# keras-team/keras-rs

Measured on AMD Instinct MI355X. Metric: embedding lookups/sec + DCN fwd+bwd step time, 26-table DLRM batch 65 536, higher is better.
Workload: dtype bf16; 1 GPU; C3 DLRM-small: 26 tables x 1000000 rows x 128 (bf16), global batch 65536, multi-hot ml_perf lengths (sum L = 214), uniform ids, DotInteraction(F=27) + 3 x FeatureCross(d=3456, projection=512), fused Adagrad on tables; global_batch=65536, parallelism=single GPU

## Files before the change

include/krs.h:

```cpp
#ifndef KRS_H_
#define KRS_H_

#include <stddef.h>
#include <stdint.h>

#ifdef __cplusplus
extern "C" {
#endif

#define KRS_VERSION 100

typedef enum krs_status {
  KRS_OK = 0,
  KRS_ERR_INVALID = -1,
  KRS_ERR_UNSUPPORTED = -2,
  KRS_ERR_LAUNCH = -3,
  KRS_ERR_WORKSPACE = -4
} krs_status;

typedef enum krs_dtype { KRS_F32 = 0, KRS_BF16 = 1 } krs_dtype;
typedef enum krs_itype { KRS_I32 = 0, KRS_I64 = 1 } krs_itype;

typedef enum krs_combiner { KRS_SUM = 0, KRS_MEAN = 1, KRS_SQRTN = 2 } krs_combiner;

// ... 147 lines not shown
enum { KRS_CROSS_BWD_NONE = 0, KRS_CROSS_BWD_TWO_CALL = 1, KRS_CROSS_BWD_PP64 = 2, KRS_CROSS_BWD_PP256 = 3 };
int krs_gemm_cross_bwd_last_route(int* epilogue);

enum {
  KRS_GEMM_KERNEL_NONE = 0, KRS_GEMM_KERNEL_GENERIC = 1, KRS_GEMM_KERNEL_MFMA = 2, KRS_GEMM_KERNEL_GLDS = 3,
  KRS_GEMM_KERNEL_TN_GLDS = 4, KRS_GEMM_KERNEL_PP256 = 5, KRS_GEMM_KERNEL_PP256_KSTRIDED = 6, KRS_GEMM_KERNEL_PP64 = 7,
  KRS_GEMM_KERNEL_THIN = 8, KRS_GEMM_KERNEL_ROWDOT = 9, KRS_GEMM_KERNEL_SMALLK = 10
};
enum { KRS_GEMM_REDUCE_NONE = 0, KRS_GEMM_REDUCE_SCALAR = 1, KRS_GEMM_REDUCE_VEC4 = 2, KRS_GEMM_REDUCE_VEC8 = 3 };
typedef struct krs_gemm_route {
  int32_t kernel;
  int32_t splits;
  int32_t reduce;
  int32_t epilogue;
  int32_t ep_vec;
  int32_t thin_width;
  int32_t thin_is_a;
} krs_gemm_route;
int krs_gemm_last_route(krs_gemm_route* route);

enum { KRS_GEMM_OPT_PIPELINE = 0 };
int krs_gemm_set_option(int key, int value);

enum { KRS_EMBED_OPT_PLAN = 2, KRS_EMBED_OPT_HOTROWS = 3, KRS_EMBED_OPT_RANK = 4 };
int krs_embed_set_option(int key, int value);

size_t krs_colsum_workspace_bytes(int64_t m, int64_t n);
int krs_cross_epilogue_fwd(const void* u, const void* x0, const void* x, void* y,
                           int64_t m, int64_t n, int64_t ld, float diag_scale,
                           int dtype, void* stream);
int krs_cross_epilogue_bwd(const void* g, const void* u, const void* x0, const void* x,
                           void* du, void* dx0, int dx0_accumulate, void* dxd,
                           float* dbias,
                           int64_t m, int64_t n, int64_t ld, float diag_scale, int act,
                           int dtype, void* workspace, size_t workspace_bytes, void* stream);

int krs_cast_transpose(const void* src, int64_t rows, int64_t cols, int64_t ld_src, int src_dtype,
                       void* dst, int64_t ld_dst, void* dst_t, int64_t ld_dst_t, int dst_dtype,
                       void* stream);
int krs_cast_transpose_many(int count, const void* const* srcs, const int64_t* rows, const int64_t* cols,
                            int src_dtype, void* const* dsts, void* const* dst_ts, int dst_dtype, void* stream);

int krs_dense_act_bwd(const void* g, int64_t ld_g, const void* y, int64_t ld_y, void* dz, int64_t ld_dz,
                      float* dbias, int64_t m, int64_t n, int act, int dtype, void* workspace,
                      size_t workspace_bytes, void* stream);

int krs_dense_adagrad(float* const* params, const float* const* grads, float* const* accs,
// ... 133 lines not shown
```

keras_rs_amd/csrc/embed_bag_fwd.hip:

```cpp
#include <cstdlib>

#include "krs_common.h"

namespace krs {
namespace {

typedef uint32_t u32x4 __attribute__((ext_vector_type(4)));
typedef float f32x4 __attribute__((ext_vector_type(4)));
constexpr int NT = 2;

struct EmbedFwdParams {
  const krs_table* tables;
  const krs_feature* feats;
  int n_feats;
  const void* ids;
  int id64;
  const void* offsets;
  int off64;
  const float* weights;
  int batch;
  int dim;
  void* out;
  int64_t out_ld;
  float* bag_scale;
// ... 522 lines not shown
      }
      KRS_CHECK_LAUNCH("embed_bag_fwd_vec (hot rows in LDS)");
      return KRS_OK;
    }
  }
  if (p.weights) { if (stream) KRS_K1_LAUNCH(true, true); else KRS_K1_LAUNCH(true, false); }
  else { if (stream) KRS_K1_LAUNCH(false, true); else KRS_K1_LAUNCH(false, false); }
#undef KRS_K1_LAUNCH
  KRS_CHECK_LAUNCH("embed_bag_fwd_vec");
  return KRS_OK;
}

template <typename TT, typename OT>
int dispatch_lpr(const EmbedFwdParams& p, int row_pieces, bool one_hot, bool stream_mode, hipStream_t stream) {
  if (row_pieces <= 8) return launch_vec<TT, OT, 8>(p, one_hot, stream_mode, stream);
  if (row_pieces <= 16) return launch_vec<TT, OT, 16>(p, one_hot, stream_mode, stream);
  if (row_pieces <= 32) return launch_vec<TT, OT, 32>(p, one_hot, stream_mode, stream);
  return launch_vec<TT, OT, 64>(p, one_hot, stream_mode, stream);
}

}
}

namespace krs { extern int g_plan_variant, g_rank_mode; }

extern "C" int krs_embed_set_option(int key, int value) {
  if (key == KRS_EMBED_OPT_PLAN) {
    KRS_REQUIRE(value == 0 || value == 1, "krs_embed_set_option: plan variant must be 0 or 1");
    krs::g_plan_variant = value;
    return KRS_OK;
  }
  if (key == KRS_EMBED_OPT_RANK) {
    KRS_REQUIRE(value >= 0 && value <= 2, "krs_embed_set_option: rank mode must be 0, 1 or 2");
    krs::g_rank_mode = value;
    return KRS_OK;
  }
  if (key == KRS_EMBED_OPT_HOTROWS) {
    KRS_REQUIRE(value == 0 || value == 64 || value == 128, "krs_embed_set_option: hot rows must be 0, 64 or 128");
    krs::g_hot_rows = value;
    return KRS_OK;
  }
  return krs::fail(KRS_ERR_INVALID, "krs_embed_set_option: unknown key %d", key);
}

extern "C" int krs_embed_bag_fwd(const krs_table* tables, const krs_feature* feats, int n_feats,
                                 const void* ids, int id_type, const void* offsets, int off_type,
                                 const float* weights, int64_t nnz, int batch, int dim,
                                 int table_dtype, void* out, int out_dtype, int64_t out_ld,
                                 float* bag_scale, int* err_flag, void* stream) {
  using namespace krs;
  KRS_REQUIRE(tables && feats && out, "embed_bag_fwd: null tables/feats/out");
  KRS_REQUIRE(ids || nnz == 0, "embed_bag_fwd: null ids");
  KRS_REQUIRE(n_feats >= 0 && batch >= 0 && dim > 0 && nnz >= 0, "embed_bag_fwd: negative size");
  KRS_REQUIRE((table_dtype == KRS_F32 || table_dtype == KRS_BF16) &&
                  (out_dtype == KRS_F32 || out_dtype == KRS_BF16),
              "embed_bag_fwd: bad dtype");
  KRS_REQUIRE((id_type == KRS_I32 || id_type == KRS_I64) && (off_type == KRS_I32 || off_type == KRS_I64),
// ... 37 lines not shown
```

keras_rs_amd/csrc/embed_bag_plan.hip:

```cpp
#include <algorithm>

#include "krs_bag_plan.h"

namespace krs {
int g_plan_variant = 0;
int g_rank_mode = 0;
namespace {

namespace rs {
constexpr int kHistThreads = 256, kHistItems = kTile / kHistThreads;
constexpr int kThreads = 512, kWaves = kThreads / 64, kItems = kTile / kThreads;
constexpr int kGenFeats = 256;

struct Gen {
  const krs_table* tables;
  const krs_feature* feats;
  int n_feats;
  const void* ids;
  int id64;
  int batch;
  int* err_flag;
};

struct alignas(16) GenLds {
  uint32_t base[kGenFeats + 1];
  uint32_t hot[kGenFeats];
  uint32_t row_base[kGenFeats];
  uint32_t vocab[kGenFeats];
};
__device__ __forceinline__ void load_gen(const Gen& gen, int64_t nnz, GenLds& g, int n_threads) {
  for (int i = threadIdx.x; i <= gen.n_feats; i += n_threads) {
    if (i < gen.n_feats) {
      const krs_feature ft = gen.feats[i];
      const krs_table tb = gen.tables[ft.table];
      g.base[i] = (uint32_t)ft.ids_base;
      g.hot[i] = (uint32_t)ft.hot;
      g.row_base[i] = (uint32_t)tb.row_base;
      g.vocab[i] = (uint32_t)tb.vocab;
    } else {
      g.base[i] = (uint32_t)nnz;
    }
  }
}
__device__ __forceinline__ int gen_feature(const GenLds& g, int n_feats, uint32_t q) {
  int lo = 0, hi = n_feats;
  while (hi - lo > 1) {
    const int mid = (lo + hi) >> 1;
    if (g.base[mid] <= q) lo = mid; else hi = mid;
  }
  return lo;
}
__device__ __forceinline__ uint64_t gen_value(const Gen& gen, const GenLds& g, int f, uint32_t q) {
  const uint32_t bag = (uint32_t)f * (uint32_t)gen.batch + (q - g.base[f]) / g.hot[f];
  return ((uint64_t)bag << 32) | (uint64_t)q;
}
__device__ __forceinline__ bool generate(const Gen& gen, const GenLds& g, uint32_t q, uint32_t& key, uint64_t& val) {
  const int f = gen_feature(g, gen.n_feats, q);
  const int64_t id = ld_index(gen.ids, gen.id64, q);
  const bool valid = id >= 0 && id < (int64_t)g.vocab[f];
  key = valid ? g.row_base[f] + (uint32_t)id : kInvalidKey;
  val = gen_value(gen, g, f, q);
  return valid;
}

__device__ __forceinline__ int digit_of(uint32_t key, int shift, int bins) { return (int)((key >> shift) & (bins - 1)); }

__device__ __forceinline__ uint32_t tile_of_block(uint32_t b, uint32_t tiles) { return (b & 7) * ((tiles + 7) / 8) + (b >> 3); }
inline unsigned tile_grid(unsigned tiles) { return (tiles + 7) / 8 * 8; }

__device__ __forceinline__ void hist_zero(int (&h)[kMaxBins], int bins) {
  for (int i = threadIdx.x; i < bins; i += kHistThreads) h[i] = 0;
}
__device__ __forceinline__ void hist_add(int (&h)[kMaxBins], uint32_t key, int shift, int bins) {
  atomicAdd(&h[digit_of(key, shift, bins)], 1);
}
__device__ __forceinline__ void hist_finish(const int (&h)[kMaxBins], int bins, int32_t* col, int64_t stride, bool bad,
                                            int* err_flag) {
  if (bad && err_flag) atomicOr(err_flag, KRS_FLAG_ID_OUT_OF_RANGE);
  __syncthreads();
  for (int i = threadIdx.x; i < bins; i += kHistThreads) col[(int64_t)i * stride] = h[i];
}

template <typename V>
struct alignas(16) TileLds {
  uint16_t cnt[kWaves][kMaxBins];
  uint16_t tile_excl[kMaxBins];
  int gbase[kMaxBins];
  uint32_t skey[kTile];
  V sval[kTile];
  int wtot[kWaves];
};
template <typename V>
__device__ __forceinline__ void zero_counts(TileLds<V>& s) {
  for (int i = threadIdx.x; i < kWaves * kMaxBins; i += kThreads) (&s.cnt[0][0])[i] = 0;
}
__device__ __forceinline__ unsigned long long digit_peers(int d, bool live, int bits) {
  unsigned long long peers = __ballot(live);
  for (int b = 0; b < bits; ++b) {
    const unsigned long long m = __ballot((d >> b) & 1);
    peers &= ((d >> b) & 1) ? m : ~m;
  }
  return peers;
}
__device__ __forceinline__ int ballot_rank(uint32_t key, bool live, int shift, int bits, volatile uint16_t* mine,
                                           int lane) {
  const int d = digit_of(key, shift, 1 << bits);
  const unsigned long long peers = digit_peers(d, live, bits);
  int r = 0, c = 0;
  if (live) {
    r = __popcll(peers & ((1ULL << lane) - 1ULL));
    const int leader = __ffsll((long long)peers) - 1;
    if (lane == leader) {
      c = mine[d];
      mine[d] = (uint16_t)(c + __popcll(peers));
    }
    c = __shfl(c, leader, 64);
  }
  __builtin_amdgcn_wave_barrier();
  return c + r;
}
typedef uint32_t __attribute__((may_alias)) cnt_word;
__device__ __forceinline__ void count_rank(const uint32_t (&key)[kItems], int64_t first, int64_t end, int shift, int bits,
                                           bool fallback, uint16_t* mine, int lane, int (&rank)[kItems]) {
  cnt_word* word = reinterpret_cast<cnt_word*>(mine);
  uint32_t before[kItems], after[kItems];
#pragma unroll
  for (int it = 0; it < kItems; ++it) {
    const int d = digit_of(key[it], shift, 1 << bits);
// ... 18 lines not shown
    if (fallback && __popcll(pend) / 2 > bits) {
      r = c + __popcll(digit_peers(d, live, bits) & below);
    } else {
      while (pend) {
        const int leader = __ffsll((long long)pend) - 1;
        const int dl = __builtin_amdgcn_readlane(d, leader);
        const unsigned long long peers = __ballot(live && d == dl);
        if (d == dl) r = c + __popcll(peers & below);
        pend &= ~peers;
      }
    }
    rank[it] = live ? r : 0;
  }
}
__device__ __forceinline__ void rank_keys(const uint32_t (&key)[kItems], int64_t first, int64_t end, int shift, int bits,
                                          int mode, uint16_t* mine, int lane, int (&rank)[kItems]) {
  if (mode == 1) {
#pragma unroll
    for (int it = 0; it < kItems; ++it) rank[it] = ballot_rank(key[it], first + it * 64 < end, shift, bits, mine, lane);
  } else {
    count_rank(key, first, end, shift, bits, mode == 0, mine, lane, rank);
  }
}
template <typename V>
__device__ __forceinline__ void digit_bases(TileLds<V>& s, int bins, const int32_t* col, int64_t stride) {
  const int lane = threadIdx.x & 63, wave = threadIdx.x >> 6;
  __syncthreads();
  int tot[2], run = 0;
#pragma unroll
  for (int k = 0; k < 2; ++k) {
    const int i = threadIdx.x * 2 + k;
    tot[k] = 0;
    if (i < bins)
      for (int w = 0; w < kWaves; ++w) tot[k] += s.cnt[w][i];
    run += tot[k];
  }
  int x = run;
#pragma unroll
  for (int o = 1; o < 64; o <<= 1) {
    const int y = __shfl_up(x, o, 64);
    if (lane >= o) x += y;
  }
  if (lane == 63) s.wtot[wave] = x;
  __syncthreads();
  int excl = x - run;
  for (int w = 0; w < wave; ++w) excl += s.wtot[w];
#pragma unroll
  for (int k = 0; k < 2; ++k) {
    const int i = threadIdx.x * 2 + k;
    if (i < bins) {
      s.tile_excl[i] = (uint16_t)excl;
      s.gbase[i] = col[(int64_t)i * stride];
      int o = excl;
      for (int w = 0; w < kWaves; ++w) {
        const int t = s.cnt[w][i];
        s.cnt[w][i] = (uint16_t)o;
        o += t;
      }
      excl += tot[k];
    }
  }
  __syncthreads();
}
template <typename V>
__device__ __forceinline__ void stage_tile(TileLds<V>& s, const uint32_t (&key)[kItems], const V (&val)[kItems],
                                           const int (&rank)[kItems], int64_t first, int64_t end, int shift, int bins) {
  const int wave = threadIdx.x >> 6;
#pragma unroll
  for (int it = 0; it < kItems; ++it) {
    if (first + it * 64 < end) {
      const int lp = s.cnt[wave][digit_of(key[it], shift, bins)] + rank[it];
      s.skey[lp] = key[it];
      s.sval[lp] = val[it];
    }
  }
  __syncthreads();
}
template <typename V>
__device__ __forceinline__ int out_slot(const TileLds<V>& s, int i, int d) {
  return s.gbase[d] + (i - (int)s.tile_excl[d]);
}

struct Pass {
  const uint32_t* keys_in;
  const uint64_t* vals_in;
  uint32_t* keys_out;
  uint64_t* vals_out;
  int32_t* counts;
  int64_t nnz;
  int n_tiles;
  int shift, bits;
  int rank;
  Gen gen;
};

template <bool GEN>
__global__ __launch_bounds__(kHistThreads) void hist_kernel(const Pass p) {
  __shared__ int h[kMaxBins];
  __shared__ GenLds g;
  const uint32_t tile = tile_of_block(blockIdx.x, p.n_tiles);
  if (tile >= (uint32_t)p.n_tiles) return;
  const int bins = 1 << p.bits;
  hist_zero(h, bins);
  if constexpr (GEN) load_gen(p.gen, p.nnz, g, kHistThreads);
  __syncthreads();
  const int64_t base = (int64_t)tile * kTile;
  bool bad = false;
  for (int it = 0; it < kHistItems; ++it) {
    const int64_t q = base + it * kHistThreads + threadIdx.x;
    if (q < p.nnz) {
      uint32_t key;
      if constexpr (GEN) {
        uint64_t v;
        bad |= !generate(p.gen, g, (uint32_t)q, key, v);
      } else {
        key = p.keys_in[q];
      }
      hist_add(h, key, p.shift, bins);
    }
  }
  hist_finish(h, bins, p.counts + tile, p.n_tiles, bad, p.gen.err_flag);
}

template <bool GEN>
__global__ __launch_bounds__(kThreads) void scatter_kernel(const Pass p) {
  __shared__ TileLds<uint64_t> s;
  __shared__ GenLds g;
  const uint32_t tile = tile_of_block(blockIdx.x, p.n_tiles);
  if (tile >= (uint32_t)p.n_tiles) return;
  const int bins = 1 << p.bits;
  zero_counts(s);
  if constexpr (GEN) load_gen(p.gen, p.nnz, g, kThreads);
  __syncthreads();
  const int lane = threadIdx.x & 63, wave = threadIdx.x >> 6;
  const int64_t tile0 = (int64_t)tile * kTile;
  const int64_t first = tile0 + (int64_t)wave * (kTile / kWaves) + lane;
  uint32_t key[kItems];
  uint64_t val[kItems];
  int rank[kItems];
#pragma unroll
  for (int it = 0; it < kItems; ++it) {
    const int64_t q = first + it * 64;
    const bool live = q < p.nnz;
    key[it] = kInvalidKey;
    val[it] = 0;
    if (live) {
      if constexpr (GEN) {
        generate(p.gen, g, (uint32_t)q, key[it], val[it]);
      } else {
        key[it] = p.keys_in[q];
        val[it] = p.vals_in[q];
      }
    }
  }
  rank_keys(key, first, p.nnz, p.shift, p.bits, p.rank, s.cnt[wave], lane, rank);
  digit_bases(s, bins, p.counts + tile, p.n_tiles);
  stage_tile(s, key, val, rank, first, p.nnz, p.shift, bins);
  const int n_here = (int)min<int64_t>(kTile, p.nnz - tile0);
#pragma unroll
  for (int it = 0; it < kItems; ++it) {
    const int i = it * kThreads + threadIdx.x;
    if (i < n_here) {
      const uint32_t k = s.skey[i];
      const int pos = out_slot(s, i, digit_of(k, p.shift, bins));
      p.keys_out[pos] = k;
      p.vals_out[pos] = s.sval[i];
    }
  }
}

struct Seg {
  int n;
  uint32_t lookup_start[kMaxProb + 1];
  uint32_t tile_start[kMaxProb + 1];
  uint32_t row_base[kMaxProb];
};
struct SegPass {
  const uint32_t* keys_in;
  const uint32_t* pos_in;
  uint32_t* keys_out;
  uint32_t* pos_out;
  uint64_t* vals_out;
  int32_t* counts;
  int64_t nnz;
  int shift, bits, key_bits;
  int rank;
  Gen gen;
  Seg seg;
};
struct SegTile {
  int pr;
  int64_t t0, end;
  int32_t* col;
  uint32_t stride;
};
__device__ __forceinline__ SegTile seg_tile(const SegPass& p, uint32_t tile) {
  const Seg& sg = p.seg;
  int lo = 0, hi = sg.n;
  while (hi - lo > 1) {
    const int mid = (lo + hi) >> 1;
    if (sg.tile_start[mid] <= tile) lo = mid; else hi = mid;
  }
  SegTile t;
  t.pr = lo;
  const uint32_t tl = tile - sg.tile_start[lo];
  t.stride = sg.tile_start[lo + 1] - sg.tile_start[lo];
  t.t0 = (int64_t)sg.lookup_start[lo] + (int64_t)tl * kTile;
  t.end = min<int64_t>(t.t0 + kTile, sg.lookup_start[lo + 1]);
  t.col = p.counts + ((int64_t)1 << p.bits) * sg.tile_start[lo] + tl;
  return t;
}
template <int ITEMS, int STRIDE>
__device__ __forceinline__ bool seg_first_keys(const SegPass& p, const GenLds& g, const SegTile& t, int64_t first,
                                               uint32_t (&key)[ITEMS], uint32_t (&pos)[ITEMS]) {
  int64_t idv[ITEMS];
#pragma unroll
  for (int it = 0; it < ITEMS; ++it) idv[it] = ld_index(p.gen.ids, p.gen.id64, min<int64_t>(first + it * STRIDE, t.end - 1));
  const int f_lo = gen_feature(g, p.gen.n_feats, (uint32_t)t.t0), f_hi = gen_feature(g, p.gen.n_feats, (uint32_t)(t.end - 1));
  bool bad = false;
#pragma unroll
  for (int it = 0; it < ITEMS; ++it) {
    const int64_t q = min<int64_t>(first + it * STRIDE, t.end - 1);
    const int f = f_lo == f_hi ? f_lo : gen_feature(g, p.gen.n_feats, (uint32_t)q);
    const bool valid = idv[it] >= 0 && idv[it] < (int64_t)g.vocab[f];
    key[it] = valid ? (uint32_t)idv[it] : (1u << p.key_bits) - 1u;
    pos[it] = (uint32_t)q;
    bad = bad || (!valid && first + it * STRIDE < t.end);
  }
  return bad;
}

template <bool FIRST>
__global__ __launch_bounds__(kHistThreads) void hist_seg_kernel(const SegPass p) {
  __shared__ int h[kMaxBins];
  __shared__ GenLds g;
  const uint32_t tile = tile_of_block(blockIdx.x, p.seg.tile_start[p.seg.n]);
  if (tile >= p.seg.tile_start[p.seg.n]) return;
  const int bins = 1 << p.bits;
  hist_zero(h, bins);
  if constexpr (FIRST) load_gen(p.gen, p.nnz, g, kHistThreads);
  __syncthreads();
  const SegTile t = seg_tile(p, tile);
  const int64_t first = t.t0 + threadIdx.x;
  bool bad = false;
  uint32_t key[kHistItems];
  if constexpr (FIRST) {
    uint32_t pos[kHistItems];
    bad = seg_first_keys<kHistItems, kHistThreads>(p, g, t, first, key, pos);
  } else {
#pragma unroll
    for (int it = 0; it < kHistItems; ++it) key[it] = p.keys_in[min<int64_t>(first + it * kHistThreads, t.end - 1)];
  }
#pragma unroll
  for (int it = 0; it < kHistItems; ++it)
    if (first + it * kHistThreads < t.end) hist_add(h, key[it], p.shift, bins);
  hist_finish(h, bins, t.col, t.stride, bad, p.gen.err_flag);
}

template <bool FIRST, bool LAST>
__global__ __launch_bounds__(kThreads) void scatter_seg_kernel(const SegPass p) {
  __shared__ TileLds<uint32_t> s;
  __shared__ GenLds g;
  const uint32_t tile = tile_of_block(blockIdx.x, p.seg.tile_start[p.seg.n]);
  if (tile >= p.seg.tile_start[p.seg.n]) return;
  const int bins = 1 << p.bits;
  zero_counts(s);
  if constexpr (FIRST || LAST) load_gen(p.gen, p.nnz, g, kThreads);
  __syncthreads();
  const int lane = threadIdx.x & 63, wave = threadIdx.x >> 6;
  const SegTile t = seg_tile(p, tile);
  const int64_t first = t.t0 + (int64_t)wave * (kTile / kWaves) + lane;
  uint32_t key[kItems], pos[kItems];
  int rank[kItems];
  if constexpr (FIRST) {
    seg_first_keys<kItems, 64>(p, g, t, first, key, pos);
  } else {
#pragma unroll
    for (int it = 0; it < kItems; ++it) {
      const int64_t q = min<int64_t>(first + it * 64, t.end - 1);
      key[it] = p.keys_in[q];
      pos[it] = p.pos_in[q];
    }
  }
#pragma unroll
  for (int it = 0; it < kItems; ++it) {
    const bool live = first + it * 64 < t.end;
    if (!live) { key[it] = 0xffffffffu; pos[it] = 0; }
  }
  rank_keys(key, first, t.end, p.shift, p.bits, p.rank, s.cnt[wave], lane, rank);
  digit_bases(s, bins, t.col, t.stride);
  stage_tile(s, key, pos, rank, first, t.end, p.shift, bins);
  const int n_here = (int)(t.end - t.t0);
  const uint32_t sentinel = (1u << p.key_bits) - 1u, rb = p.seg.row_base[t.pr];
  int pf_lo = 0, pf_hi = 1;
  if constexpr (LAST) {
    pf_lo = gen_feature(g, p.gen.n_feats, p.seg.lookup_start[t.pr]);
    pf_hi = gen_feature(g, p.gen.n_feats, p.seg.lookup_start[t.pr + 1] - 1);
  }
// ... 38 lines not shown
inline Gen make_gen(const krs_table* tables, const krs_feature* feats, int n_feats, const void* ids, int id_type,
                    int batch, int* err_flag) {
  Gen g;
  g.tables = tables; g.feats = feats; g.n_feats = n_feats; g.ids = ids;
  g.id64 = id_type == KRS_I64; g.batch = batch; g.err_flag = err_flag;
  return g;
}
}

struct KeyParams {
  const krs_table* tables;
  const krs_feature* feats;
  int n_feats;
  const void* ids;
  int id64;
  const void* offsets;
  int off64;
  int batch;
  uint32_t* keys;
  uint64_t* vals;
  int* err_flag;
};

__global__ __launch_bounds__(256) void bag_keys_kernel(const KeyParams p) {
  const int64_t bag = (int64_t)blockIdx.x * 16 + (threadIdx.x >> 4);
  const int sub = threadIdx.x & 15;
  if (bag >= (int64_t)p.n_feats * p.batch) return;
  const int f = (int)(bag / p.batch);
  const int b = (int)(bag - (int64_t)f * p.batch);
  const krs_feature ft = p.feats[f];
  const krs_table tb = p.tables[ft.table];
  int64_t s, e;
  if (p.offsets) {
    s = ld_index(p.offsets, p.off64, bag);
    e = ld_index(p.offsets, p.off64, bag + 1);
  } else {
    s = ft.ids_base + (int64_t)b * ft.hot;
    e = s + ft.hot;
  }
  int oob = 0;
  for (int64_t q = s + sub; q < e; q += 16) {
    const int64_t id = ld_index(p.ids, p.id64, q);
    uint32_t key = kInvalidKey;
    if (id >= 0 && id < tb.vocab)
      key = (uint32_t)(tb.row_base + id);
    else
      oob = 1;
    p.keys[q] = key;
    p.vals[q] = ((uint64_t)bag << 32) | (uint64_t)(uint32_t)q;
  }
  if (oob && p.err_flag) atomicOr(p.err_flag, KRS_FLAG_ID_OUT_OF_RANGE);
}

constexpr int kSegTile = 4096, kSegItems = 16;
__device__ __forceinline__ uint32_t seg_head_mask(const uint32_t* keys, int64_t nnz, int64_t t0) {
  if (t0 >= nnz) return 0u;
  uint32_t prev = t0 > 0 ? keys[t0 - 1] : ~keys[0];
  uint32_t mask = 0u;
  if (t0 + kSegItems <= nnz) {
    const uint4* v = reinterpret_cast<const uint4*>(keys + t0);
#pragma unroll
    for (int q = 0; q < kSegItems / 4; ++q) {
      const uint4 k = v[q];
      mask |= (uint32_t)(k.x != prev) << (4 * q);
      mask |= (uint32_t)(k.y != k.x) << (4 * q + 1);
      mask |= (uint32_t)(k.z != k.y) << (4 * q + 2);
      mask |= (uint32_t)(k.w != k.z) << (4 * q + 3);
      prev = k.w;
    }
  } else {
    for (int k = 0; t0 + k < nnz; ++k) {
      const uint32_t cur = keys[t0 + k];
      mask |= (uint32_t)(cur != prev) << k;
// ... 34 lines not shown
    m &= m - 1;
    seg_start[off++] = (uint32_t)(t0 + k);
  }
  if (t0 < nnz && t0 + kSegItems >= nnz) *n_seg = off;
}
__global__ void long_list_kernel(const uint32_t* seg_start, const uint32_t* n_seg, int64_t nnz, uint32_t* counters,
                                 LongItem* items, MultiSeg* multi) {
  const int64_t u = (int64_t)blockIdx.x * blockDim.x + threadIdx.x;
  const uint32_t ns = *n_seg;
  if (u >= ns) return;
  const int64_t e = u + 1 < ns ? (int64_t)seg_start[u + 1] : nnz;
  const int64_t len = e - (int64_t)seg_start[u];
  if (len <= kLongSeg) return;
  const uint32_t nch = (uint32_t)((len + kChunk - 1) / kChunk);
  const uint32_t base = atomicAdd(counters, nch);
  uint32_t pb = 0xffffffffu;
  if (nch > 1) {
    pb = atomicAdd(counters + 1, nch);
    multi[atomicAdd(counters + 2, 1u)] = MultiSeg{(uint32_t)u, pb, nch};
  }
  for (uint32_t c = 0; c < nch; ++c) items[base + c] = LongItem{(uint32_t)u, c, nch > 1 ? pb + c : 0xffffffffu};
}

bool plan_sort_by_table(const PlanLayout& l, const rs::Temp& tmp, const rs::Gen& gen, const krs_table* tables_host,
                        int n_tables, const krs_feature* feats_host, int64_t nnz, hipStream_t st) {
  if (!tables_host || !feats_host || gen.n_feats > rs::kGenFeats || n_tables <= 0) return false;
  rs::SegPass sp;
  rs::Seg& sg = sp.seg;
  sg.n = 0;
  int64_t pos = 0, max_vocab = 0;
  int prev_table = -1;
  for (int f = 0; f < gen.n_feats; ++f) {
    const krs_feature& ft = feats_host[f];
    if (ft.hot < 1 || ft.ids_base != pos || ft.table < prev_table || ft.table >= n_tables) return false;
    if (ft.table != prev_table) {
      if (sg.n == rs::kMaxProb) return false;
      const krs_table& tb = tables_host[ft.table];
      if (prev_table >= 0 && tb.row_base < tables_host[prev_table].row_base + tables_host[prev_table].vocab) return false;
      sg.lookup_start[sg.n] = (uint32_t)pos;
      sg.row_base[sg.n] = (uint32_t)tb.row_base;
      max_vocab = std::max<int64_t>(max_vocab, tb.vocab);
      ++sg.n;
      prev_table = ft.table;
    }
    pos += (int64_t)gen.batch * ft.hot;
  }
  if (pos != nnz || sg.n == 0) return false;
  sg.lookup_start[sg.n] = (uint32_t)nnz;
  uint32_t tiles = 0;
  for (int i = 0; i < sg.n; ++i) {
    sg.tile_start[i] = tiles;
    tiles += (uint32_t)ceil_div((int64_t)sg.lookup_start[i + 1] - sg.lookup_start[i], rs::kTile);
  }
  sg.tile_start[sg.n] = tiles;
  if (tiles == 0) return false;
  const unsigned bits = rs::key_bits(max_vocab);
  if (bits > 31) return false;
  const rs::Schedule sch = rs::pass_schedule(bits);
  sp.counts = tmp.counts; sp.nnz = nnz; sp.key_bits = (int)bits; sp.rank = g_rank_mode;
  sp.gen = gen;
  uint32_t* k0 = l.keys_in; uint32_t* q0 = reinterpret_cast<uint32_t*>(l.vals_in);
  uint32_t* k1 = l.keys_sorted; uint32_t* q1 = reinterpret_cast<uint32_t*>(l.vals_sorted);
  for (int ps = 0; ps < sch.passes; ++ps) {
    const bool first = ps == 0, last = ps == sch.passes - 1;
    sp.bits = sch.bits[ps];
    sp.shift = sch.shift[ps];
    const bool out_is_i0 = ((sch.passes - 2 - ps) % 2) == 0;
    const bool in_is_i0 = ((sch.passes - 1 - ps) % 2) == 0;
    sp.keys_in = first ? nullptr : (in_is_i0 ? k0 : k1);
    sp.pos_in = first ? nullptr : (in_is_i0 ? q0 : q1);
    sp.keys_out = last ? l.keys_sorted : (out_is_i0 ? k0 : k1);
    sp.pos_out = last ? nullptr : (out_is_i0 ? q0 : q1);
    sp.vals_out = last ? l.vals_sorted : nullptr;
    if (first) hipLaunchKernelGGL(rs::hist_seg_kernel<true>, dim3(rs::tile_grid(tiles)), dim3(rs::kHistThreads), 0, st, sp);
    else hipLaunchKernelGGL(rs::hist_seg_kernel<false>, dim3(rs::tile_grid(tiles)), dim3(rs::kHistThreads), 0, st, sp);
    scan::exclusive(tmp.counts, tmp.counts, (int64_t)(1 << sp.bits) * tiles, tmp.sums, nullptr, st);
    if (first && last) hipLaunchKernelGGL((rs::scatter_seg_kernel<true, true>), dim3(rs::tile_grid(tiles)), dim3(rs::kThreads), 0, st, sp);
    else if (first) hipLaunchKernelGGL((rs::scatter_seg_kernel<true, false>), dim3(rs::tile_grid(tiles)), dim3(rs::kThreads), 0, st, sp);
    else if (last) hipLaunchKernelGGL((rs::scatter_seg_kernel<false, true>), dim3(rs::tile_grid(tiles)), dim3(rs::kThreads), 0, st, sp);
    else hipLaunchKernelGGL((rs::scatter_seg_kernel<false, false>), dim3(rs::tile_grid(tiles)), dim3(rs::kThreads), 0, st, sp);
  }
  return true;
}

int plan_sort_global(const PlanLayout& l, const rs::Temp& tmp, const rs::Gen& gen, const void* offsets, int off_type,
                     int64_t nnz, int64_t total_rows, hipStream_t st) {
  const rs::Schedule sch = rs::pass_schedule(rs::key_bits(total_rows));
  const bool gen_first = offsets == nullptr && gen.n_feats <= rs::kGenFeats;
  bool to_sorted = (sch.passes % 2) == 1;
  if (!gen_first) {
    KeyParams kp;
    kp.tables = gen.tables; kp.feats = gen.feats; kp.n_feats = gen.n_feats; kp.ids = gen.ids; kp.id64 = gen.id64;
    kp.offsets = offsets; kp.off64 = off_type == KRS_I64; kp.batch = gen.batch; kp.err_flag = gen.err_flag;
    kp.keys = to_sorted ? l.keys_in : l.keys_sorted;
    kp.vals = to_sorted ? l.vals_in : l.vals_sorted;
    const int64_t n_bags = (int64_t)gen.n_feats * gen.batch;
    KRS_HIP(hipMemsetAsync(kp.keys, 0xff, (size_t)nnz * sizeof(uint32_t), st));
    hipLaunchKernelGGL(bag_keys_kernel, dim3((unsigned)ceil_div(n_bags, 16)), dim3(256), 0, st, kp);
    KRS_CHECK_LAUNCH("bag_keys_kernel");
  }
  rs::Pass p;
  p.nnz = nnz;
  p.n_tiles = (int)ceil_div(nnz, rs::kTile);
  p.counts = tmp.counts;
  p.rank = g_rank_mode;
  p.gen = gen;
  for (int ps = 0; ps < sch.passes; ++ps) {
    p.bits = sch.bits[ps];
    p.shift = sch.shift[ps];
    const bool generating = gen_first && ps == 0;
    p.keys_in = generating ? nullptr : (to_sorted ? l.keys_in : l.keys_sorted);
    p.vals_in = generating ? nullptr : (to_sorted ? l.vals_in : l.vals_sorted);
    p.keys_out = to_sorted ? l.keys_sorted : l.keys_in;
    p.vals_out = to_sorted ? l.vals_sorted : l.vals_in;
    if (generating) hipLaunchKernelGGL(rs::hist_kernel<true>, dim3(rs::tile_grid((unsigned)p.n_tiles)), dim3(rs::kHistThreads), 0, st, p);
    else hipLaunchKernelGGL(rs::hist_kernel<false>, dim3(rs::tile_grid((unsigned)p.n_tiles)), dim3(rs::kHistThreads), 0, st, p);
    scan::exclusive(tmp.counts, tmp.counts, (int64_t)(1 << p.bits) * p.n_tiles, tmp.sums, nullptr, st);
    if (generating) hipLaunchKernelGGL(rs::scatter_kernel<true>, dim3(rs::tile_grid((unsigned)p.n_tiles)), dim3(rs::kThreads), 0, st, p);
    else hipLaunchKernelGGL(rs::scatter_kernel<false>, dim3(rs::tile_grid((unsigned)p.n_tiles)), dim3(rs::kThreads), 0, st, p);
    to_sorted = !to_sorted;
  }
  return KRS_OK;
}

int plan_impl(const krs_table* tables, const krs_table* tables_host, int n_tables, const krs_feature* feats,
              const krs_feature* feats_host, int n_feats, const void* ids, int id_type, const void* offsets,
              int off_type, int batch, int64_t nnz, int64_t total_rows, void* workspace, size_t workspace_bytes,
              int* err_flag, void* stream) {
  KRS_REQUIRE(tables && feats && (ids || nnz == 0), "embed_bag_bwd_plan: null argument");
  KRS_REQUIRE(n_feats > 0 && batch > 0 && nnz >= 0, "embed_bag_bwd_plan: bad sizes");
  KRS_REQUIRE(total_rows > 0 && total_rows < 0xffffffffLL, "embed_bag_bwd_plan: total_rows must fit 32-bit keys");
  KRS_REQUIRE(nnz < 0x7fffffffLL && (int64_t)n_feats * batch < 0xffffffffLL,
              "embed_bag_bwd_plan: nnz must stay below 2^31 and the bag count below 2^32");
  if (nnz == 0) return KRS_OK;
  KRS_REQUIRE(workspace, "embed_bag_bwd_plan: null workspace");
  const PlanLayout l = plan_layout(workspace, nnz, true);
  if (workspace_bytes < l.total_bytes)
    return fail(KRS_ERR_WORKSPACE, "embed_bag_bwd_plan: workspace %zu < %zu bytes", workspace_bytes, l.total_bytes);
  hipStream_t st = reinterpret_cast<hipStream_t>(stream);
  const rs::Temp tmp = rs::carve_temp(l.temp, nnz);
  const rs::Gen gen = rs::make_gen(tables, feats, n_feats, ids, id_type, batch, err_flag);
  const bool by_table = offsets == nullptr && g_plan_variant == 0 &&
                        plan_sort_by_table(l, tmp, gen, tables_host, n_tables, feats_host, nnz, st);
  if (!by_table)
    if (int rc = plan_sort_global(l, tmp, gen, offsets, off_type, nnz, total_rows, st)) return rc;
  KRS_CHECK_LAUNCH("embed_bag_bwd_plan: radix sort");
  const unsigned nb = (unsigned)ceil_div(nnz, 256);
  const unsigned nsb = (unsigned)ceil_div(nnz, kSegTile);
  hipLaunchKernelGGL(seg_count_kernel, dim3(nsb), dim3(256), 0, st, l.keys_sorted, nnz, tmp.sums2);
  hipLaunchKernelGGL(scan::block_kernel, dim3(1), dim3(1024), 0, st, tmp.sums2, (int64_t)nsb, (int64_t*)nullptr);
  hipLaunchKernelGGL(seg_emit_kernel, dim3(nsb), dim3(256), 0, st, l.keys_sorted, nnz, tmp.sums2, l.seg_start, l.n_seg);
  KRS_CHECK_LAUNCH("seg_emit_kernel");
  KRS_HIP(hipMemsetAsync(l.n_long, 0, 3 * sizeof(uint32_t), st));
  KRS_HIP(hipMemsetAsync(l.sort_mode, by_table ? 1 : 0, sizeof(uint32_t), st));
  hipLaunchKernelGGL(long_list_kernel, dim3(nb), dim3(256), 0, st, l.seg_start, l.n_seg, nnz, l.n_long, l.long_list,
                     l.multi_list);
  KRS_CHECK_LAUNCH("long_list_kernel");
  return KRS_OK;
}

}
}

using namespace krs;

extern "C" size_t krs_embed_bag_bwd_workspace_bytes(int64_t nnz) {
// ... 21 lines not shown
```

keras_rs_amd/csrc/krs_common.h:

```cpp
#ifndef KRS_COMMON_H_
#define KRS_COMMON_H_

#include <hip/hip_runtime.h>
#include <stdint.h>

#include <cstdarg>
#include <cstdio>

#include "../../include/krs.h"

namespace krs {

char* error_buffer();
inline int fail(int code, const char* fmt, ...) {
  va_list ap;
  va_start(ap, fmt);
  vsnprintf(error_buffer(), 512, fmt, ap);
  va_end(ap);
  return code;
}

#define KRS_REQUIRE(cond, ...)                                   \
  do {                                                           \
    if (!(cond)) return ::krs::fail(KRS_ERR_INVALID, __VA_ARGS__); \
// ... 27 lines not shown
__device__ __forceinline__ float load1(const T* p) {
  if constexpr (sizeof(T) == 2) return bf16_to_f32(*p);
  else return *p;
}
template <typename T>
__device__ __forceinline__ void store1(T* p, float v) {
  if constexpr (sizeof(T) == 2) *p = f32_to_bf16(v);
  else *p = v;
}
__device__ __forceinline__ float quiet_nan() { return __uint_as_float(0x7fc00000u); }

__device__ __forceinline__ float ld_elem(const void* p, int dtype, int64_t i) {
  return dtype == KRS_BF16 ? bf16_to_f32(((const uint16_t*)p)[i]) : ((const float*)p)[i];
}
__device__ __forceinline__ void st_elem(void* p, int dtype, int64_t i, float v) {
  if (dtype == KRS_BF16)
    ((uint16_t*)p)[i] = f32_to_bf16(v);
  else
    ((float*)p)[i] = v;
}
__device__ __forceinline__ int64_t ld_index(const void* p, int is64, int64_t i) {
  return is64 ? ((const int64_t*)p)[i] : (int64_t)((const int32_t*)p)[i];
}

__device__ __forceinline__ uint32_t order_key(float f) {
  uint32_t u = __float_as_uint(f);
  if ((u & 0x7fffffffu) > 0x7f800000u) return 0xffffffffu;
  if (u == 0x80000000u) u = 0;
  return (u & 0x80000000u) ? ~u : (u | 0x80000000u);
}

__host__ __device__ __forceinline__ int64_t ceil_div(int64_t a, int64_t b) { return (a + b - 1) / b; }
template <typename I>
__host__ __device__ __forceinline__ I pow2_at_least(I v) {
  I p = 1;
  while (p < v) p <<= 1;
  return p;
}

}
#endif
```

Measured before the change: 1.496 billion lookups/s.

## Template radix-sort tile geometry and default by-table plan sort to wide tiles

```diff
diff --git a/include/krs.h b/include/krs.h
--- a/include/krs.h
+++ b/include/krs.h
@@ -193,7 +193,7 @@
 enum { KRS_GEMM_OPT_PIPELINE = 0 };
 int krs_gemm_set_option(int key, int value);
 
-enum { KRS_EMBED_OPT_PLAN = 2, KRS_EMBED_OPT_HOTROWS = 3, KRS_EMBED_OPT_RANK = 4 };
+enum { KRS_EMBED_OPT_PLAN = 2, KRS_EMBED_OPT_HOTROWS = 3, KRS_EMBED_OPT_RANK = 4, KRS_EMBED_OPT_TILE = 5 };
 int krs_embed_set_option(int key, int value);
 
 size_t krs_colsum_workspace_bytes(int64_t m, int64_t n);
diff --git a/keras_rs_amd/csrc/embed_bag_fwd.hip b/keras_rs_amd/csrc/embed_bag_fwd.hip
--- a/keras_rs_amd/csrc/embed_bag_fwd.hip
+++ b/keras_rs_amd/csrc/embed_bag_fwd.hip
@@ -568,7 +568,7 @@
 }
 }
 
-namespace krs { extern int g_plan_variant, g_rank_mode; }
+namespace krs { extern int g_plan_variant, g_rank_mode, g_plan_tile; }
 
 extern "C" int krs_embed_set_option(int key, int value) {
   if (key == KRS_EMBED_OPT_PLAN) {
@@ -579,6 +579,11 @@
   if (key == KRS_EMBED_OPT_RANK) {
     KRS_REQUIRE(value >= 0 && value <= 2, "krs_embed_set_option: rank mode must be 0, 1 or 2");
     krs::g_rank_mode = value;
+    return KRS_OK;
+  }
+  if (key == KRS_EMBED_OPT_TILE) {
+    KRS_REQUIRE(value == 4096 || value == 8192, "krs_embed_set_option: tile must be 4096 or 8192");
+    krs::g_plan_tile = value;
     return KRS_OK;
   }
   if (key == KRS_EMBED_OPT_HOTROWS) {
diff --git a/keras_rs_amd/csrc/embed_bag_plan.hip b/keras_rs_amd/csrc/embed_bag_plan.hip
--- a/keras_rs_amd/csrc/embed_bag_plan.hip
+++ b/keras_rs_amd/csrc/embed_bag_plan.hip
@@ -5,11 +5,15 @@
 namespace krs {
 int g_plan_variant = 0;
 int g_rank_mode = 0;
+int g_plan_tile = 8192;
 namespace {
 
 namespace rs {
-constexpr int kHistThreads = 256, kHistItems = kTile / kHistThreads;
-constexpr int kThreads = 512, kWaves = kThreads / 64, kItems = kTile / kThreads;
+constexpr int kItems = 8, kHistItems = 16;
+template <int W>
+struct Geo {
+  static constexpr int kWaves = W, kTile = 512 * W, kThreads = 64 * W, kHistThreads = 32 * W;
+};
 constexpr int kGenFeats = 256;
 
 struct Gen {
@@ -54,9 +58,9 @@
   const uint32_t bag = (uint32_t)f * (uint32_t)gen.batch + (q - g.base[f]) / g.hot[f];
   return ((uint64_t)bag << 32) | (uint64_t)q;
 }
-__device__ __forceinline__ bool generate(const Gen& gen, const GenLds& g, uint32_t q, uint32_t& key, uint64_t& val) {
+__device__ __forceinline__ bool generate(const Gen& gen, const GenLds& g, uint32_t q, int64_t id, uint32_t& key,
+                                         uint64_t& val) {
   const int f = gen_feature(g, gen.n_feats, q);
-  const int64_t id = ld_index(gen.ids, gen.id64, q);
   const bool valid = id >= 0 && id < (int64_t)g.vocab[f];
   key = valid ? g.row_base[f] + (uint32_t)id : kInvalidKey;
   val = gen_value(gen, g, f, q);
@@ -68,21 +72,24 @@
 __device__ __forceinline__ uint32_t tile_of_block(uint32_t b, uint32_t tiles) { return (b & 7) * ((tiles + 7) / 8) + (b >> 3); }
 inline unsigned tile_grid(unsigned tiles) { return (tiles + 7) / 8 * 8; }
 
+template <int HT>
 __device__ __forceinline__ void hist_zero(int (&h)[kMaxBins], int bins) {
-  for (int i = threadIdx.x; i < bins; i += kHistThreads) h[i] = 0;
+  for (int i = threadIdx.x; i < bins; i += HT) h[i] = 0;
 }
 __device__ __forceinline__ void hist_add(int (&h)[kMaxBins], uint32_t key, int shift, int bins) {
   atomicAdd(&h[digit_of(key, shift, bins)], 1);
 }
+template <int HT>
 __device__ __forceinline__ void hist_finish(const int (&h)[kMaxBins], int bins, int32_t* col, int64_t stride, bool bad,
                                             int* err_flag) {
   if (bad && err_flag) atomicOr(err_flag, KRS_FLAG_ID_OUT_OF_RANGE);
   __syncthreads();
-  for (int i = threadIdx.x; i < bins; i += kHistThreads) col[(int64_t)i * stride] = h[i];
-}
-
-template <typename V>
+  for (int i = threadIdx.x; i < bins; i += HT) col[(int64_t)i * stride] = h[i];
+}
+
+template <typename V, int W>
 struct alignas(16) TileLds {
+  static constexpr int kWaves = W, kTile = 512 * W, kThreads = 64 * W;
   uint16_t cnt[kWaves][kMaxBins];
   uint16_t tile_excl[kMaxBins];
   int gbase[kMaxBins];
@@ -90,9 +97,9 @@
   V sval[kTile];
   int wtot[kWaves];
 };
-template <typename V>
-__device__ __forceinline__ void zero_counts(TileLds<V>& s) {
-  for (int i = threadIdx.x; i < kWaves * kMaxBins; i += kThreads) (&s.cnt[0][0])[i] = 0;
+template <typename S>
+__device__ __forceinline__ void zero_counts(S& s) {
+  for (int i = threadIdx.x; i < S::kWaves * kMaxBins; i += S::kThreads) (&s.cnt[0][0])[i] = 0;
 }
 __device__ __forceinline__ unsigned long long digit_peers(int d, bool live, int bits) {
   unsigned long long peers = __ballot(live);
@@ -102,8 +109,9 @@
   }
   return peers;
 }
-__device__ __forceinline__ int ballot_rank(uint32_t key, bool live, int shift, int bits, volatile uint16_t* mine,
-                                           int lane) {
+typedef __attribute__((address_space(3))) uint16_t lds_u16;
+__device__ __forceinline__ int ballot_rank(uint32_t key, bool live, int shift, int bits, uint16_t* cnt_row, int lane) {
+  volatile lds_u16* mine = (volatile lds_u16*)cnt_row;
   const int d = digit_of(key, shift, 1 << bits);
   const unsigned long long peers = digit_peers(d, live, bits);
   int r = 0, c = 0;
@@ -168,8 +176,9 @@
     count_rank(key, first, end, shift, bits, mode == 0, mine, lane, rank);
   }
 }
-template <typename V>
-__device__ __forceinline__ void digit_bases(TileLds<V>& s, int bins, const int32_t* col, int64_t stride) {
+template <typename S>
+__device__ __forceinline__ void digit_bases(S& s, int bins, const int32_t* col, int64_t stride) {
+  constexpr int kWaves = S::kWaves;
   const int lane = threadIdx.x & 63, wave = threadIdx.x >> 6;
   __syncthreads();
   int tot[2], run = 0;
@@ -208,8 +217,8 @@
   }
   __syncthreads();
 }
-template <typename V>
-__device__ __forceinline__ void stage_tile(TileLds<V>& s, const uint32_t (&key)[kItems], const V (&val)[kItems],
+template <typename S, typename V>
+__device__ __forceinline__ void stage_tile(S& s, const uint32_t (&key)[kItems], const V (&val)[kItems],
                                            const int (&rank)[kItems], int64_t first, int64_t end, int shift, int bins) {
   const int wave = threadIdx.x >> 6;
 #pragma unroll
@@ -222,8 +231,8 @@
   }
   __syncthreads();
 }
-template <typename V>
-__device__ __forceinline__ int out_slot(const TileLds<V>& s, int i, int d) {
+template <typename S>
+__device__ __forceinline__ int out_slot(const S& s, int i, int d) {
   return s.gbase[d] + (i - (int)s.tile_excl[d]);
 }
 
@@ -240,37 +249,44 @@
   Gen gen;
 };
 
-template <bool GEN>
-__global__ __launch_bounds__(kHistThreads) void hist_kernel(const Pass p) {
+template <int W, bool GEN, bool ID64>
+__global__ __launch_bounds__(Geo<W>::kHistThreads) void hist_kernel(const Pass p) {
+  constexpr int kTile = Geo<W>::kTile, kHistThreads = Geo<W>::kHistThreads;
   __shared__ int h[kMaxBins];
   __shared__ GenLds g;
   const uint32_t tile = tile_of_block(blockIdx.x, p.n_tiles);
   if (tile >= (uint32_t)p.n_tiles) return;
   const int bins = 1 << p.bits;
-  hist_zero(h, bins);
+  hist_zero<kHistThreads>(h, bins);
   if constexpr (GEN) load_gen(p.gen, p.nnz, g, kHistThreads);
   __syncthreads();
-  const int64_t base = (int64_t)tile * kTile;
+  const int64_t first = (int64_t)tile * kTile + threadIdx.x, last = p.nnz - 1;
   bool bad = false;
-  for (int it = 0; it < kHistItems; ++it) {
-    const int64_t q = base + it * kHistThreads + threadIdx.x;
-    if (q < p.nnz) {
-      uint32_t key;
-      if constexpr (GEN) {
-        uint64_t v;
-        bad |= !generate(p.gen, g, (uint32_t)q, key, v);
-      } else {
-        key = p.keys_in[q];
-      }
-      hist_add(h, key, p.shift, bins);
-    }
-  }
-  hist_finish(h, bins, p.counts + tile, p.n_tiles, bad, p.gen.err_flag);
-}
-
-template <bool GEN>
-__global__ __launch_bounds__(kThreads) void scatter_kernel(const Pass p) {
-  __shared__ TileLds<uint64_t> s;
+  uint32_t key[kHistItems];
+  if constexpr (GEN) {
+    int64_t idv[kHistItems];
+    ld_indices<kHistItems, kHistThreads>(p.gen.ids, ID64, first, last, idv);
+#pragma unroll
+    for (int it = 0; it < kHistItems; ++it) {
+      const int64_t q = first + it * kHistThreads;
+      uint64_t v;
+      const bool valid = generate(p.gen, g, (uint32_t)min<int64_t>(q, last), idv[it], key[it], v);
+      bad = bad || (!valid && q <= last);
+    }
+  } else {
+#pragma unroll
+    for (int it = 0; it < kHistItems; ++it) key[it] = p.keys_in[min<int64_t>(first + it * kHistThreads, last)];
+  }
+#pragma unroll
+  for (int it = 0; it < kHistItems; ++it)
+    if (first + it * kHistThreads <= last) hist_add(h, key[it], p.shift, bins);
+  hist_finish<kHistThreads>(h, bins, p.counts + tile, p.n_tiles, bad, p.gen.err_flag);
+}
+
+template <int W, bool GEN, bool ID64>
+__global__ __launch_bounds__(Geo<W>::kThreads) void scatter_kernel(const Pass p) {
+  constexpr int kTile = Geo<W>::kTile, kThreads = Geo<W>::kThreads, kWaves = W;
+  __shared__ TileLds<uint64_t, W> s;
   __shared__ GenLds g;
   const uint32_t tile = tile_of_block(blockIdx.x, p.n_tiles);
   if (tile >= (uint32_t)p.n_tiles) return;
@@ -284,21 +300,24 @@
   uint32_t key[kItems];
   uint64_t val[kItems];
   int rank[kItems];
-#pragma unroll
-  for (int it = 0; it < kItems; ++it) {
-    const int64_t q = first + it * 64;
-    const bool live = q < p.nnz;
-    key[it] = kInvalidKey;
-    val[it] = 0;
-    if (live) {
-      if constexpr (GEN) {
-        generate(p.gen, g, (uint32_t)q, key[it], val[it]);
-      } else {
-        key[it] = p.keys_in[q];
-        val[it] = p.vals_in[q];
-      }
-    }
-  }
+  const int64_t last = p.nnz - 1;
+  if constexpr (GEN) {
+    int64_t idv[kItems];
+    ld_indices<kItems, 64>(p.gen.ids, ID64, first, last, idv);
+#pragma unroll
+    for (int it = 0; it < kItems; ++it)
+      generate(p.gen, g, (uint32_t)min<int64_t>(first + it * 64, last), idv[it], key[it], val[it]);
+  } else {
+#pragma unroll
+    for (int it = 0; it < kItems; ++it) {
+      const int64_t q = min<int64_t>(first + it * 64, last);
+      key[it] = p.keys_in[q];
+      val[it] = p.vals_in[q];
+    }
+  }
+#pragma unroll
+  for (int it = 0; it < kItems; ++it)
+    if (first + it * 64 > last) { key[it] = kInvalidKey; val[it] = 0; }
   rank_keys(key, first, p.nnz, p.shift, p.bits, p.rank, s.cnt[wave], lane, rank);
   digit_bases(s, bins, p.counts + tile, p.n_tiles);
   stage_tile(s, key, val, rank, first, p.nnz, p.shift, bins);
@@ -340,6 +359,7 @@
   int32_t* col;
   uint32_t stride;
 };
+template <int kTile>
 __device__ __forceinline__ SegTile seg_tile(const SegPass& p, uint32_t tile) {
   const Seg& sg = p.seg;
   int lo = 0, hi = sg.n;
@@ -356,12 +376,11 @@
   t.col = p.counts + ((int64_t)1 << p.bits) * sg.tile_start[lo] + tl;
   return t;
 }
-template <int ITEMS, int STRIDE>
+template <int ITEMS, int STRIDE, bool ID64>
 __device__ __forceinline__ bool seg_first_keys(const SegPass& p, const GenLds& g, const SegTile& t, int64_t first,
                                                uint32_t (&key)[ITEMS], uint32_t (&pos)[ITEMS]) {
   int64_t idv[ITEMS];
-#pragma unroll
-  for (int it = 0; it < ITEMS; ++it) idv[it] = ld_index(p.gen.ids, p.gen.id64, min<int64_t>(first + it * STRIDE, t.end - 1));
+  ld_indices<ITEMS, STRIDE>(p.gen.ids, ID64, first, t.end - 1, idv);
   const int f_lo = gen_feature(g, p.gen.n_feats, (uint32_t)t.t0), f_hi = gen_feature(g, p.gen.n_feats, (uint32_t)(t.end - 1));
   bool bad = false;
 #pragma unroll
@@ -376,23 +395,24 @@
   return bad;
 }
 
-template <bool FIRST>
-__global__ __launch_bounds__(kHistThreads) void hist_seg_kernel(const SegPass p) {
+template <int W, bool FIRST, bool ID64>
+__global__ __launch_bounds__(Geo<W>::kHistThreads) void hist_seg_kernel(const SegPass p) {
+  constexpr int kTile = Geo<W>::kTile, kHistThreads = Geo<W>::kHistThreads;
   __shared__ int h[kMaxBins];
   __shared__ GenLds g;
   const uint32_t tile = tile_of_block(blockIdx.x, p.seg.tile_start[p.seg.n]);
   if (tile >= p.seg.tile_start[p.seg.n]) return;
   const int bins = 1 << p.bits;
-  hist_zero(h, bins);
+  hist_zero<kHistThreads>(h, bins);
   if constexpr (FIRST) load_gen(p.gen, p.nnz, g, kHistThreads);
   __syncthreads();
-  const SegTile t = seg_tile(p, tile);
+  const SegTile t = seg_tile<kTile>(p, tile);
   const int64_t first = t.t0 + threadIdx.x;
   bool bad = false;
   uint32_t key[kHistItems];
   if constexpr (FIRST) {
     uint32_t pos[kHistItems];
-    bad = seg_first_keys<kHistItems, kHistThreads>(p, g, t, first, key, pos);
+    bad = seg_first_keys<kHistItems, kHistThreads, ID64>(p, g, t, first, key, pos);
   } else {
 #pragma unroll
     for (int it = 0; it < kHistItems; ++it) key[it] = p.keys_in[min<int64_t>(first + it * kHistThreads, t.end - 1)];
@@ -400,12 +420,13 @@
 #pragma unroll
   for (int it = 0; it < kHistItems; ++it)
     if (first + it * kHistThreads < t.end) hist_add(h, key[it], p.shift, bins);
-  hist_finish(h, bins, t.col, t.stride, bad, p.gen.err_flag);
-}
-
-template <bool FIRST, bool LAST>
-__global__ __launch_bounds__(kThreads) void scatter_seg_kernel(const SegPass p) {
-  __shared__ TileLds<uint32_t> s;
+  hist_finish<kHistThreads>(h, bins, t.col, t.stride, bad, p.gen.err_flag);
+}
+
+template <int W, bool FIRST, bool LAST, bool ID64>
+__global__ __launch_bounds__(Geo<W>::kThreads) void scatter_seg_kernel(const SegPass p) {
+  constexpr int kTile = Geo<W>::kTile, kThreads = Geo<W>::kThreads, kWaves = W;
+  __shared__ TileLds<uint32_t, W> s;
   __shared__ GenLds g;
   const uint32_t tile = tile_of_block(blockIdx.x, p.seg.tile_start[p.seg.n]);
   if (tile >= p.seg.tile_start[p.seg.n]) return;
@@ -414,12 +435,12 @@
   if constexpr (FIRST || LAST) load_gen(p.gen, p.nnz, g, kThreads);
   __syncthreads();
   const int lane = threadIdx.x & 63, wave = threadIdx.x >> 6;
-  const SegTile t = seg_tile(p, tile);
+  const SegTile t = seg_tile<kTile>(p, tile);
   const int64_t first = t.t0 + (int64_t)wave * (kTile / kWaves) + lane;
   uint32_t key[kItems], pos[kItems];
   int rank[kItems];
   if constexpr (FIRST) {
-    seg_first_keys<kItems, 64>(p, g, t, first, key, pos);
+    seg_first_keys<kItems, 64, ID64>(p, g, t, first, key, pos);
   } else {
 #pragma unroll
     for (int it = 0; it < kItems; ++it) {
@@ -504,6 +525,23 @@
   int* err_flag;
 };
 
+template <bool ID64>
+__device__ __forceinline__ int bag_keys(const KeyParams& p, int64_t row_base, int64_t vocab, int64_t bag, int64_t q, int64_t e) {
+  int oob = 0;
+  for (; q < e; q += 16) {
+    int64_t id;
+    if constexpr (ID64) id = ((const int64_t*)p.ids)[q];
+    else id = ((const int32_t*)p.ids)[q];
+    uint32_t key = kInvalidKey;
+    if (id >= 0 && id < vocab)
+      key = (uint32_t)(row_base + id);
+    else
+      oob = 1;
+    p.keys[q] = key;
+    p.vals[q] = ((uint64_t)bag << 32) | (uint64_t)(uint32_t)q;
+  }
+  return oob;
+}
 __global__ __launch_bounds__(256) void bag_keys_kernel(const KeyParams p) {
   const int64_t bag = (int64_t)blockIdx.x * 16 + (threadIdx.x >> 4);
   const int sub = threadIdx.x & 15;
@@ -514,23 +552,16 @@
   const krs_table tb = p.tables[ft.table];
   int64_t s, e;
   if (p.offsets) {
-    s = ld_index(p.offsets, p.off64, bag);
-    e = ld_index(p.offsets, p.off64, bag + 1);
+    int64_t se[2];
+    ld_indices<2, 1>(p.offsets, p.off64, bag, bag + 1, se);
+    s = se[0];
+    e = se[1];
   } else {
     s = ft.ids_base + (int64_t)b * ft.hot;
     e = s + ft.hot;
   }
-  int oob = 0;
-  for (int64_t q = s + sub; q < e; q += 16) {
-    const int64_t id = ld_index(p.ids, p.id64, q);
-    uint32_t key = kInvalidKey;
-    if (id >= 0 && id < tb.vocab)
-      key = (uint32_t)(tb.row_base + id);
-    else
-      oob = 1;
-    p.keys[q] = key;
-    p.vals[q] = ((uint64_t)bag << 32) | (uint64_t)(uint32_t)q;
-  }
+  const int oob = p.id64 ? bag_keys<true>(p, tb.row_base, tb.vocab, bag, s + sub, e)
+                         : bag_keys<false>(p, tb.row_base, tb.vocab, bag, s + sub, e);
   if (oob && p.err_flag) atomicOr(p.err_flag, KRS_FLAG_ID_OUT_OF_RANGE);
 }
 
@@ -611,6 +642,7 @@
   for (uint32_t c = 0; c < nch; ++c) items[base + c] = LongItem{(uint32_t)u, c, nch > 1 ? pb + c : 0xffffffffu};
 }
 
+template <int W>
 bool plan_sort_by_table(const PlanLayout& l, const rs::Temp& tmp, const rs::Gen& gen, const krs_table* tables_host,
                         int n_tables, const krs_feature* feats_host, int64_t nnz, hipStream_t st) {
   if (!tables_host || !feats_host || gen.n_feats > rs::kGenFeats || n_tables <= 0) return false;
@@ -639,7 +671,7 @@
   uint32_t tiles = 0;
   for (int i = 0; i < sg.n; ++i) {
     sg.tile_start[i] = tiles;
-    tiles += (uint32_t)ceil_div((int64_t)sg.lookup_start[i + 1] - sg.lookup_start[i], rs::kTile);
+    tiles += (uint32_t)ceil_div((int64_t)sg.lookup_start[i + 1] - sg.lookup_start[i], rs::Geo<W>::kTile);
   }
   sg.tile_start[sg.n] = tiles;
   if (tiles == 0) return false;
@@ -661,19 +693,26 @@
     sp.keys_out = last ? l.keys_sorted : (out_is_i0 ? k0 : k1);
     sp.pos_out = last ? nullptr : (out_is_i0 ? q0 : q1);
     sp.vals_out = last ? l.vals_sorted : nullptr;
-    if (first) hipLaunchKernelGGL(rs::hist_seg_kernel<true>, dim3(rs::tile_grid(tiles)), dim3(rs::kHistThreads), 0, st, sp);
-    else hipLaunchKernelGGL(rs::hist_seg_kernel<false>, dim3(rs::tile_grid(tiles)), dim3(rs::kHistThreads), 0, st, sp);
+    const dim3 grid(rs::tile_grid(tiles));
+    void (*hist)(rs::SegPass) = rs::hist_seg_kernel<W, false, false>;
+    void (*scatter)(rs::SegPass) = last ? rs::scatter_seg_kernel<W, false, true, false> : rs::scatter_seg_kernel<W, false, false, false>;
+    if (first && gen.id64) {
+      hist = rs::hist_seg_kernel<W, true, true>;
+      scatter = last ? rs::scatter_seg_kernel<W, true, true, true> : rs::scatter_seg_kernel<W, true, false, true>;
+    } else if (first) {
+      hist = rs::hist_seg_kernel<W, true, false>;
+      scatter = last ? rs::scatter_seg_kernel<W, true, true, false> : rs::scatter_seg_kernel<W, true, false, false>;
+    }
+    hipLaunchKernelGGL(hist, grid, dim3(rs::Geo<W>::kHistThreads), 0, st, sp);
     scan::exclusive(tmp.counts, tmp.counts, (int64_t)(1 << sp.bits) * tiles, tmp.sums, nullptr, st);
-    if (first && last) hipLaunchKernelGGL((rs::scatter_seg_kernel<true, true>), dim3(rs::tile_grid(tiles)), dim3(rs::kThreads), 0, st, sp);
-    else if (first) hipLaunchKernelGGL((rs::scatter_seg_kernel<true, false>), dim3(rs::tile_grid(tiles)), dim3(rs::kThreads), 0, st, sp);
-    else if (last) hipLaunchKernelGGL((rs::scatter_seg_kernel<false, true>), dim3(rs::tile_grid(tiles)), dim3(rs::kThreads), 0, st, sp);
-    else hipLaunchKernelGGL((rs::scatter_seg_kernel<false, false>), dim3(rs::tile_grid(tiles)), dim3(rs::kThreads), 0, st, sp);
+    hipLaunchKernelGGL(scatter, grid, dim3(rs::Geo<W>::kThreads), 0, st, sp);
   }
   return true;
 }
 
 int plan_sort_global(const PlanLayout& l, const rs::Temp& tmp, const rs::Gen& gen, const void* offsets, int off_type,
                      int64_t nnz, int64_t total_rows, hipStream_t st) {
+  constexpr int W = 8;
   const rs::Schedule sch = rs::pass_schedule(rs::key_bits(total_rows));
   const bool gen_first = offsets == nullptr && gen.n_feats <= rs::kGenFeats;
   bool to_sorted = (sch.passes % 2) == 1;
@@ -690,7 +729,7 @@
   }
   rs::Pass p;
   p.nnz = nnz;
-  p.n_tiles = (int)ceil_div(nnz, rs::kTile);
+  p.n_tiles = (int)ceil_div(nnz, rs::Geo<W>::kTile);
   p.counts = tmp.counts;
   p.rank = g_rank_mode;
   p.gen = gen;
@@ -702,11 +741,16 @@
     p.vals_in = generating ? nullptr : (to_sorted ? l.vals_in : l.vals_sorted);
     p.keys_out = to_sorted ? l.keys_sorted : l.keys_in;
     p.vals_out = to_sorted ? l.vals_sorted : l.vals_in;
-    if (generating) hipLaunchKernelGGL(rs::hist_kernel<true>, dim3(rs::tile_grid((unsigned)p.n_tiles)), dim3(rs::kHistThreads), 0, st, p);
-    else hipLaunchKernelGGL(rs::hist_kernel<false>, dim3(rs::tile_grid((unsigned)p.n_tiles)), dim3(rs::kHistThreads), 0, st, p);
+    const dim3 grid(rs::tile_grid((unsigned)p.n_tiles));
+    void (*hist)(rs::Pass) = rs::hist_kernel<W, false, false>;
+    void (*scatter)(rs::Pass) = rs::scatter_kernel<W, false, false>;
+    if (generating) {
+      hist = gen.id64 ? rs::hist_kernel<W, true, true> : rs::hist_kernel<W, true, false>;
+      scatter = gen.id64 ? rs::scatter_kernel<W, true, true> : rs::scatter_kernel<W, true, false>;
+    }
+    hipLaunchKernelGGL(hist, grid, dim3(rs::Geo<W>::kHistThreads), 0, st, p);
     scan::exclusive(tmp.counts, tmp.counts, (int64_t)(1 << p.bits) * p.n_tiles, tmp.sums, nullptr, st);
-    if (generating) hipLaunchKernelGGL(rs::scatter_kernel<true>, dim3(rs::tile_grid((unsigned)p.n_tiles)), dim3(rs::kThreads), 0, st, p);
-    else hipLaunchKernelGGL(rs::scatter_kernel<false>, dim3(rs::tile_grid((unsigned)p.n_tiles)), dim3(rs::kThreads), 0, st, p);
+    hipLaunchKernelGGL(scatter, grid, dim3(rs::Geo<W>::kThreads), 0, st, p);
     to_sorted = !to_sorted;
   }
   return KRS_OK;
@@ -729,8 +773,10 @@
   hipStream_t st = reinterpret_cast<hipStream_t>(stream);
   const rs::Temp tmp = rs::carve_temp(l.temp, nnz);
   const rs::Gen gen = rs::make_gen(tables, feats, n_feats, ids, id_type, batch, err_flag);
+  const bool wide = g_plan_tile == 8192;
   const bool by_table = offsets == nullptr && g_plan_variant == 0 &&
-                        plan_sort_by_table(l, tmp, gen, tables_host, n_tables, feats_host, nnz, st);
+                        (wide ? plan_sort_by_table<16>(l, tmp, gen, tables_host, n_tables, feats_host, nnz, st)
+                              : plan_sort_by_table<8>(l, tmp, gen, tables_host, n_tables, feats_host, nnz, st));
   if (!by_table)
     if (int rc = plan_sort_global(l, tmp, gen, offsets, off_type, nnz, total_rows, st)) return rc;
   KRS_CHECK_LAUNCH("embed_bag_bwd_plan: radix sort");
diff --git a/keras_rs_amd/csrc/krs_common.h b/keras_rs_amd/csrc/krs_common.h
--- a/keras_rs_amd/csrc/krs_common.h
+++ b/keras_rs_amd/csrc/krs_common.h
@@ -73,6 +73,18 @@
 __device__ __forceinline__ int64_t ld_index(const void* p, int is64, int64_t i) {
   return is64 ? ((const int64_t*)p)[i] : (int64_t)((const int32_t*)p)[i];
 }
+template <int N, int STRIDE>
+__device__ __forceinline__ void ld_indices(const void* p, int is64, int64_t first, int64_t last, int64_t (&out)[N]) {
+  if (is64) {
+    const int64_t* src = (const int64_t*)p;
+#pragma unroll
+    for (int k = 0; k < N; ++k) { const int64_t i = first + (int64_t)k * STRIDE; out[k] = src[i < last ? i : last]; }
+  } else {
+    const int32_t* src = (const int32_t*)p;
+#pragma unroll
+    for (int k = 0; k < N; ++k) { const int64_t i = first + (int64_t)k * STRIDE; out[k] = (int64_t)src[i < last ? i : last]; }
+  }
+}
 
 __device__ __forceinline__ uint32_t order_key(float f) {
   uint32_t u = __float_as_uint(f);
```

Measured after the change: 1.506 billion lookups/s, median of 6. No clear change (+0.7%).
